# isl-org/adaptive-surface-reconstruction

Hardware: AMD Instinct MI355X
Metric: input points/sec to signed implicit values (higher is better)
Workload: dtype f32 via bf16x3 (24-bit operands, f32 accumulate)

## Files before the change

### adaptive-surface-reconstruction_amd/csrc/asr_common.h

```cpp
#pragma once
#include <hip/hip_runtime.h>

#include <cstdint>
#include <cstdio>
#include <map>
#include <string>
#include <tuple>
#include <vector>

#include "../../include/asr_hip.h"

typedef uint64_t u64;
typedef int64_t i64;
typedef uint32_t u32;

struct Arena {
    struct Slab {
        char* base;
        size_t size, used;
    };
    std::vector<Slab> slabs;
    size_t min_slab = size_t(256) << 20;
    size_t cap = 0;

// ... 44 lines not shown
    float* centers = nullptr;
    float* sizes = nullptr;
    int32_t* nidx = nullptr;
    uint8_t* nkidx = nullptr;
    i64* nrs = nullptr;
    int32_t* up_idx = nullptr;
    uint8_t* up_kidx = nullptr;
    i64* up_rs = nullptr;
    int32_t* down_idx = nullptr;
    uint8_t* down_kidx = nullptr;
    i64* down_rs = nullptr;
    int32_t* perm_nb = nullptr;
    int32_t* perm_up = nullptr;
    int32_t* perm_down = nullptr;
};

struct AsrOptions {
    i64 sconv_min_blocks = 2816;
    i64 sconv16_min_blocks = 1024;
    i64 sconv_wide_min = 2048;
    i64 row_segment = 524288;
    i64 search_hash_level = -1;
    i64 knn_deep = 1;
    i64 knn_cells = 1;
    i64 plan_arena = 0;
    i64 sconv_plan = 1;
    i64 row_ranked = 1;
    i64 row_lpt = 1;
    i64 overlap = 1;
    i64 cconv_valu = 0;
    i64 build_search = 1;
    i64 shard_geometry = -1;
    i64 shard_timing = 0;
    i64 search_priority = 2;
    i64 search_half = 1;
    i64 early_cells = 1;
    i64 early_sort = 1;
    i64 arena_cap_mb = 0;
    i64 inject_failure = 0;
    i64 sconv_split_min_rows = 2048;
    i64 sconv_split_rows = 32768;
};

struct asr_conv_plan_view {
    const uint4* hdr;
    const int32_t* pool;
    i64 groups;
    unsigned pool_bytes;
};
struct asr_conv_plan {
    uint4* hdr = nullptr;
    int32_t* pool = nullptr;
    i64 groups = 0, groups_pad = 0, blocks = 0;
    i64* offs = nullptr;
    const int32_t* nidx = nullptr;
    const uint8_t* kidx = nullptr;
    const i64* rs = nullptr;
    const int32_t* perm = nullptr;
    i64 num_out = 0;
    int K = 0;
    bool usable() const { return hdr && blocks * 64 < (i64(1) << 32) - 65536; }
    asr_conv_plan_view view() const { return {hdr, pool, groups, (unsigned)(blocks * 64)}; }
};

struct AsrPointIndex {
    bool valid = false;
    const float* pts = nullptr;
    const float* radii = nullptr;
    i64 n = 0;
    int lsort = 0;
    float4* sorted = nullptr;
    int32_t* ids = nullptr;
    int32_t* rank = nullptr;
    float* srad = nullptr;
    u64* codes = nullptr;
    u64* tab_keys = nullptr;
    u64 tab_mask = 0;
    int32_t* tab_start = nullptr;
    int32_t* tab_end = nullptr;
    int tab_lmin = 0, tab_lmax = -1, tab_lhash = 0, tab_grow = 0;
};

struct asr_hip_context {
    hipStream_t stream = nullptr;
    std::string err;
    AsrOptions opt;
    std::map<const void*, asr_conv_plan> conv_plans;
    std::map<std::string, i64> sconv_launches;
    ArenaMark build_mark;
    bool build_mark_ok = false;
    Arena persist;
    Arena scratch;
    Arena plan_arena;
    uint64_t plan_arena_epoch = 0;
    u64* nodes = nullptr;
    u64* leaves = nullptr;
    i64 num_nodes = 0, num_leaves = 0;
    asr_octree_frame frame;
    asr_implicit_sizes sizes;
    GridDev grids[ASR_NUM_GRIDS];
    int32_t* agg_idx = nullptr;
    float* agg_dist = nullptr;
    float* agg_compat = nullptr;
    i64* agg_rs = nullptr;
    int32_t* agg_spos = nullptr;
    const float4* agg_sorted = nullptr;
    bool has_search = false;
    bool build_sharded = false;
    const int32_t* agg_rows = nullptr;
    i64 agg_nq = 0;
    const float* agg_qcenters = nullptr;
    const float* agg_qsizes = nullptr;
// ... 293 lines not shown
```

### adaptive-surface-reconstruction_amd/csrc/asr_geom.hip

```cpp
#include <cstdlib>
#include <cstring>
#include <algorithm>
#include <rocprim/rocprim.hpp>

#include "asr_common.h"
#include "asr_prim.h"

namespace {
using namespace asr_prim;

constexpr int BLK = 256;

struct HashTab {
    u64* keys;
    int32_t* vals;
    u64 mask;
};

struct TabProbe {
    u64 bucket, step, low, bmask;
    __device__ inline u64 slot() const { return ((bucket & bmask) << 6) | low; }
    __device__ inline void next() { bucket += step; }
};
__device__ inline TabProbe tab_probe(const HashTab& t, u64 key) {
// ... 598 lines not shown
__global__ void k_gather_radii(const float* radii, const int32_t* ids, i64 n, float* out) {
    i64 i = blockIdx.x * (i64)blockDim.x + threadIdx.x;
    if (i < n) out[i] = radii[ids[i]];
}
__device__ inline int query_level(const asr_octree_frame& f, float r) {
    int lev = 0;
    while (lev < ASR_MAX_LEVEL && f.voxel_size[lev + 1] >= r) ++lev;
    return lev;
}
__global__ __launch_bounds__(256) void k_query_levels(asr_octree_frame f, const float* sizes, i64 v, int* cnt) {
    __shared__ int s_lo[4], s_hi[4];
    int lo = ASR_MAX_LEVEL, hi = 0;
    for (i64 i = blockIdx.x * (i64)blockDim.x + threadIdx.x; i < v; i += (i64)gridDim.x * blockDim.x) {
        const int l = query_level(f, sizes[i]);
        lo = min(lo, l);
        hi = max(hi, l);
    }
#pragma unroll
    for (int o = 32; o > 0; o >>= 1) {
        lo = min(lo, __shfl_xor(lo, o, 64));
        hi = max(hi, __shfl_xor(hi, o, 64));
    }
    if ((threadIdx.x & 63) == 0) {
        s_lo[threadIdx.x >> 6] = lo;
        s_hi[threadIdx.x >> 6] = hi;
    }
    __syncthreads();
    if (threadIdx.x == 0) {
        atomicMin(&cnt[6], min(min(s_lo[0], s_lo[1]), min(s_lo[2], s_lo[3])));
        atomicMax(&cnt[7], max(max(s_hi[0], s_hi[1]), max(s_hi[2], s_hi[3])));
    }
}
template <bool COUNT_ONLY>
__global__ __launch_bounds__(256) void k_cell_bounds(const u64* codes, i64 n, int lmin, int lmax, HashTab t,
                                                     int32_t* start, int32_t* end, int* cnt, int* level_cnt) {
    __shared__ int s_sum[4];
    __shared__ int s_lvl[ASR_MAX_LEVEL + 1];
    if (COUNT_ONLY) {
        if (threadIdx.x <= ASR_MAX_LEVEL) s_lvl[threadIdx.x] = 0;
        __syncthreads();
    }
    int local = 0;
    for (i64 i = blockIdx.x * (i64)blockDim.x + threadIdx.x; i <= n; i += (i64)gridDim.x * blockDim.x) {
        u64 a = i > 0 ? codes[i - 1] : 0, b = i < n ? codes[i] : 0;
        for (int l = lmin; l <= lmax; ++l) {
            int s = 3 * (ASR_MAX_LEVEL - l);
            u64 pa = (s >= 63) ? 0 : (a >> s), pb = (s >= 63) ? 0 : (b >> s);
            bool has_a = i > 0, has_b = i < n;
            if (has_a && has_b && pa == pb) continue;
            u64 marker = u64(1) << (3 * l);
            if (COUNT_ONLY) {
                if (has_b) {
                    ++local;
                    atomicAdd(&s_lvl[l], 1);
                }
            } else {
                u64 slot;
                if (has_a) {
                    if (tab_insert(t, pa | marker, &slot) < 0)
                        cnt[1] = 1;
                    else
                        end[slot] = (int32_t)i;
                }
                if (has_b) {
                    if (tab_insert(t, pb | marker, &slot) < 0)
                        cnt[1] = 1;
                    else
                        start[slot] = (int32_t)i;
                }
            }
        }
    }
    if (COUNT_ONLY) {
#pragma unroll
        for (int o = 32; o > 0; o >>= 1) local += __shfl_xor(local, o, 64);
        if ((threadIdx.x & 63) == 0) s_sum[threadIdx.x >> 6] = local;
        __syncthreads();
        if (threadIdx.x == 0) atomicAdd(&cnt[8], s_sum[0] + s_sum[1] + s_sum[2] + s_sum[3]);
        if (level_cnt && threadIdx.x <= ASR_MAX_LEVEL && s_lvl[threadIdx.x]) atomicAdd(&level_cnt[threadIdx.x], s_lvl[threadIdx.x]);
    }
}

__device__ inline float sqdist3(float ax, float ay, float az, float bx, float by, float bz) {
    float dx = ax - bx, dy = ay - by, dz = az - bz;
    float s = dx * dx;
    s = s + dy * dy;
    s = s + dz * dz;
    return s;
}

constexpr int RADIUS_LIGHT = 128;
constexpr int RADIUS_GIANT = 4096;
constexpr int RADIUS_SPLIT = 64;

struct CellIndex {
    HashTab tab;
    const int32_t* start;
    const int32_t* end;
    const u64* codes;
    int n;
    int lhash;
};
__device__ inline void cell_range(const CellIndex& ci, u64 cell, int lev, int& b, int& cnt) {
    b = 0;
    cnt = 0;
    if (lev <= ci.lhash) {
        const i64 slot = tab_find_slot(ci.tab, cell | (u64(1) << (3 * lev)));
        if (slot >= 0) {
            b = ci.start[slot];
            cnt = ci.end[slot] - b;
        }
        return;
    }
    const int s = 3 * (ASR_MAX_LEVEL - lev);
    int lo = 0, hi = ci.n;
    while (lo < hi) {
        const int mid = (lo + hi) >> 1;
        if ((ci.codes[mid] >> s) < cell)
            lo = mid + 1;
        else
            hi = mid;
    }
    int lo2 = lo, hi2 = ci.n;
    while (lo2 < hi2) {
        const int mid = (lo2 + hi2) >> 1;
        if ((ci.codes[mid] >> s) <= cell)
            lo2 = mid + 1;
        else
            hi2 = mid;
    }
    b = lo;
    cnt = lo2 - lo;
}

template <int NCELL>
__device__ inline int cells_prefix(int b, int n, int lane, int* s_pref, int* s_beg) {
    int pre = n;
#pragma unroll
    for (int o = 1; o < (NCELL > 32 ? 64 : 32); o <<= 1) {
        int up = __shfl_up(pre, o, 64);
        if (lane >= o) pre += up;
    }
    if (lane < NCELL) {
        s_pref[lane + 1] = pre;
        s_beg[lane] = b;
    }
    if (lane == 0) s_pref[0] = 0;
    const int total = __shfl(pre, NCELL - 1, 64);
    __builtin_amdgcn_wave_barrier();
    return total;
}
__device__ inline int radius_cells(const asr_octree_frame& f, const CellIndex& ci, float cx, float cy, float cz,
                                   float r, int lane, int* s_pref, int* s_beg) {
    const int lev = query_level(f, r);
    int x, y, z;
    frame_coord(f, cx, cy, cz, lev, x, y, z);
    const int lim = (1 << lev) - 1;
    int b = 0, n = 0;
    if (lane < 27) {
        int xx = x + lane % 3 - 1, yy = y + (lane / 3) % 3 - 1, zz = z + lane / 9 - 1;
        if (xx >= 0 && yy >= 0 && zz >= 0 && xx <= lim && yy <= lim && zz <= lim)
            cell_range(ci, asr_morton3d((u64)xx, (u64)yy, (u64)zz), lev, b, n);
    }
    return cells_prefix<27>(b, n, lane, s_pref, s_beg);
}

constexpr int EXTRA_CAP = 1 << 16;
struct AlignedQ {
    const u64* keys;
    const int2* extras;
    const int* extras_cnt;
    int lhalf_max;
};
__device__ inline int aligned_cells(const CellIndex& ci, const AlignedQ& aq, u64 key, int lane, int* s_pref, int* s_beg) {
    int x, y, z, lev;
    asr_key_coord(key, x, y, z, lev);
    int b = 0, n = 0;
    if (lev <= aq.lhalf_max) {
        const int lim = (2 << lev) - 1;
        const int xx = 2 * x - 1 + (lane & 3), yy = 2 * y - 1 + ((lane >> 2) & 3), zz = 2 * z - 1 + (lane >> 4);
        if (xx >= 0 && yy >= 0 && zz >= 0 && xx <= lim && yy <= lim && zz <= lim)
            cell_range(ci, asr_morton3d((u64)xx, (u64)yy, (u64)zz), lev + 1, b, n);
    } else if (lane < 27) {
        const int lim = (1 << lev) - 1;
        const int xx = x + lane % 3 - 1, yy = y + (lane / 3) % 3 - 1, zz = z + lane / 9 - 1;
        if (xx >= 0 && yy >= 0 && zz >= 0 && xx <= lim && yy <= lim && zz <= lim)
            cell_range(ci, asr_morton3d((u64)xx, (u64)yy, (u64)zz), lev, b, n);
    }
    return cells_prefix<64>(b, n, lane, s_pref, s_beg);
}
template <int NCELL = 27>
__device__ inline float4 radius_candidate(const float4* sorted, const int* s_pref, const int* s_beg, int i,
                                          int* pos_out = nullptr) {
    int lo = 0, hi = NCELL;
    while (hi - lo > 1) {
        int mid = (lo + hi) >> 1;
        if (s_pref[mid] <= i)
            lo = mid;
        else
            hi = mid;
    }
    const int pos = s_beg[lo] + (i - s_pref[lo]);
    if (pos_out) *pos_out = pos;
    return sorted[pos];
}

struct ExtraParams {
    int lmin, lmax;
    int T;
    int rho[ASR_MAX_LEVEL + 1];
};
__global__ void k_radius_extras(const u64* codes, const float4* sorted, i64 n, const u64* keys, i64 v, const float* centers,
                                const float* sizes, ExtraParams ep, int2* out, int* out_cnt) {
    const i64 s = blockIdx.x * (i64)blockDim.x + threadIdx.x;
    if (s >= n) return;
// ... 642 lines not shown
                            const int i = i0 + lane;
                            bool b2 = false;
                            if (i < total) {
                                const float4 pt = cand_pt(i);
                                b2 = __float_as_uint(sqdist3(pt.x, pt.y, pt.z, me.x, me.y, me.z)) == kth_bits &&
                                     (u32)__float_as_int(pt.w) < trial;
                            }
                            below += __popcll(__ballot(b2));
                        }
                        if (below < admit) idx_hi = trial;
                    }
                    votes_eq = 0;
                    for (int i0 = 0; i0 < total; i0 += 64) {
                        const int i = i0 + lane;
                        bool v = false;
                        if (i < total) {
                            const float4 pt = cand_pt(i);
                            v = __float_as_uint(sqdist3(pt.x, pt.y, pt.z, me.x, me.y, me.z)) == kth_bits &&
                                (u32)__float_as_int(pt.w) <= idx_hi && radii_in[__float_as_int(pt.w)] < thr;
                        }
                        votes_eq += __popcll(__ballot(v));
                    }
                }
                const int votes = votes_lt + votes_eq;
                if (lane == 0) inlier_out[__float_as_int(me.w)] = votes < outlier_threshold ? 1 : 0;
            }
            break;
        }
    }
    if (lane == 0 && radii_out) radii_out[__float_as_int(me.w)] = sqrtf(__uint_as_float(kth_bits));
}


__global__ void k_max_cell_pop(HashTab t, const int32_t* start, const int32_t* end, int level, int* out) {
    const u64 slot = blockIdx.x * (u64)blockDim.x + threadIdx.x;
    if (slot > t.mask) return;
    const u64 key = t.keys[slot];
    if (key == 0 || asr_key_level(key) != level) return;
    const int pop = end[slot] - start[slot];
    if (pop > KNN_CROWD) atomicMax(out, pop);
}

__global__ __launch_bounds__(256) void k_cell_list(const u64* codes, i64 n, int level, int32_t* list, int* cnt) {
    __shared__ int s_cnt[256];
    __shared__ int s_base;
    const int s = 3 * (ASR_MAX_LEVEL - level);
    const i64 base = blockIdx.x * (i64)4096;
    int mine = 0;
    unsigned flags = 0;
#pragma unroll
    for (int j = 0; j < 16; ++j) {
        const i64 i = base + j * 256 + threadIdx.x;
        if (i < n && (i == 0 || (codes[i - 1] >> s) != (codes[i] >> s))) {
            flags |= 1u << j;
            ++mine;
        }
    }
    s_cnt[threadIdx.x] = mine;
    __syncthreads();
    if (threadIdx.x == 0) {
        int tot = 0;
        for (int t = 0; t < 256; ++t) {
            const int c = s_cnt[t];
            s_cnt[t] = tot;
            tot += c;
        }
        s_base = tot ? atomicAdd(cnt, tot) : 0;
    }
    __syncthreads();
    int o = s_base + s_cnt[threadIdx.x];
#pragma unroll
    for (int j = 0; j < 16; ++j)
        if (flags & (1u << j)) list[o++] = (int32_t)(base + j * 256 + threadIdx.x);
}

constexpr int KNN_CELL_MAX_WORK = 12288;
template <int K>
__global__ __launch_bounds__(256) void k_knn_cells(asr_octree_frame f, const float4* sorted, i64 n, HashTab t,
                                                   const int32_t* start, const int32_t* end, int lfine, int k,
                                                   const int32_t* cells, i64 ncells, float* radii_out,
                                                   int32_t* fallback, int* fallback_cnt) {
    __shared__ int s_pref[4][28];
    __shared__ int s_beg[4][28];
    __shared__ __attribute__((aligned(16))) float4 s_cand[4][64];
    const int lane = threadIdx.x & 63, wave = threadIdx.x >> 6;
    const i64 ci = blockIdx.x * (i64)4 + wave;
    if (ci >= ncells) return;
    const int first = cells[ci];
    const float4 p0 = sorted[first];
    int x, y, z;
    frame_coord(f, p0.x, p0.y, p0.z, lfine, x, y, z);
    const int lim = (1 << lfine) - 1;
    x = min(max(x, 0), lim);
    y = min(max(y, 0), lim);
    z = min(max(z, 0), lim);
    int b = 0, cnt = 0;
    if (lane < 27) {
        constexpr unsigned char order[27] = {13, 4, 10, 12, 14, 16, 22, 1, 3, 5, 7, 9, 11, 15, 17, 19, 21, 23, 25,
                                             0, 2, 6, 8, 18, 20, 24, 26};
        const int c = order[lane];
        int xx = x + c % 3 - 1, yy = y + (c / 3) % 3 - 1, zz = z + c / 9 - 1;
        if (xx >= 0 && yy >= 0 && zz >= 0 && xx <= lim && yy <= lim && zz <= lim) {
            i64 slot = tab_find_slot(t, asr_morton3d((u64)xx, (u64)yy, (u64)zz) | (u64(1) << (3 * lfine)));
            if (slot >= 0) {
                b = start[slot];
                cnt = end[slot] - b;
            }
        }
    }
    int pre = cnt;
#pragma unroll
    for (int o = 1; o < 32; o <<= 1) {
        int up = __shfl_up(pre, o, 64);
        if (lane >= o) pre += up;
    }
    const int total = __shfl(pre, 26, 64);
    const int qb = __shfl(b, 0, 64), qn = __shfl(cnt, 0, 64);
    if (lane < 27) {
        s_pref[wave][lane + 1] = pre;
        s_beg[wave][lane] = b;
    }
    if (lane == 0) s_pref[wave][0] = 0;
    __builtin_amdgcn_wave_barrier();
    const float cs = f.voxel_size[lfine];
    const float cs2 = cs * cs;
    if (total < k || (i64)((qn + 63) / 64) * total > KNN_CELL_MAX_WORK) {
        for (int q0 = lane; q0 < qn; q0 += 64) fallback[atomicAdd(fallback_cnt, 1)] = qb + q0;
        return;
    }
    for (int q0 = 0; q0 < qn; q0 += 64) {
        const bool active = q0 + lane < qn;
        const float4 me = sorted[qb + (active ? q0 + lane : 0)];
        float a[K];
#pragma unroll
        for (int c = 0; c < K; ++c) a[c] = __uint_as_float(0x7f800000u);
        if (total >= k) {
            for (int c0 = 0; c0 < total; c0 += 64) {
                const int m = min(64, total - c0);
                __builtin_amdgcn_wave_barrier();
// ... 863 lines not shown
    *out_keys = arena_alloc<u64>(keep, vo);
    *up_idx = arena_alloc<int32_t>(keep, v);
    *up_kidx = arena_alloc<uint8_t>(keep, v);
    *up_rs = arena_alloc<i64>(keep, v + 1);
    *down_idx = arena_alloc<int32_t>(keep, v);
    *down_kidx = arena_alloc<uint8_t>(keep, v);
    *down_rs = arena_alloc<i64>(keep, vo + 1);
    if (!src || !*out_keys || !*up_idx || !*up_kidx || !*up_rs || !*down_idx || !*down_kidx || !*down_rs)
        ASR_FAIL(ctx, ASR_HIP_EHIP, "arena allocation failed");
    return coarsen_lists(ctx, keys, v, pre, vo, src, *out_keys, *up_idx, *up_kidx, *up_rs, *down_idx, *down_kidx,
                         *down_rs);
}

int asr_geom_voxel_info(asr_hip_context* ctx, const asr_octree_frame* frame, const u64* keys,
                        i64 v, float* centers, float* sizes) {
    if (v <= 0) return ASR_HIP_OK;
    k_voxel_info<<<grid_for(v, BLK), BLK, 0, ctx->stream>>>(*frame, keys, v, centers, sizes);
    ASR_CHECK_LAUNCH(ctx);
    return ASR_HIP_OK;
}

struct RadiusState {
    bool valid = false;
    asr_octree_frame frame;
    float4* sorted = nullptr;
    int32_t* ids = nullptr;
    int32_t* rank = nullptr;
    const u64* codes = nullptr;
    u64* codes_w = nullptr;
    const u64* codes_u = nullptr;
    const int32_t* ids_u = nullptr;
    int32_t* ids_w = nullptr;
    int lhash = ASR_MAX_LEVEL;
    CellIndex index() const { return {tab, start, end, codes, (int)n, lhash}; }
    HashTab tab;
    int32_t* start = nullptr;
    int32_t* end = nullptr;
    i64 n = 0, v = 0;
    u64* tmp = nullptr;
    int32_t* heavy = nullptr;
    uint8_t* is_heavy = nullptr;
    i64 num_heavy = 0;
    int* hc_pref = nullptr;
    int* hc_beg = nullptr;
    const u64* dual_leaves = nullptr;
    i64 dual_nl = 0;
    float* srad = nullptr;
    const float* radii_src = nullptr;
    int lsort = 0;
    int cell_grow = 0;
    bool aligned = false;
    bool aligned_main = false;
    AlignedQ aq = {nullptr, nullptr, nullptr, -1};
};
static RadiusState& rstate(asr_hip_context* ctx) {
    if (!ctx->radius_state) ctx->radius_state = new RadiusState();
    return *(RadiusState*)ctx->radius_state;
}
void asr_geom_release(asr_hip_context* ctx) {
    delete (RadiusState*)ctx->radius_state;
    ctx->radius_state = nullptr;
}

static int sort_points(asr_hip_context* ctx, const asr_octree_frame* frame, const float* pts, i64 n, int lsort,
                       RadiusState& st, Arena* keep, bool want_rank, const float* radii, bool keep_all = false) {
    st.frame = *frame;
    st.n = n;
    st.lsort = lsort;
    Arena& ka = keep ? *keep : ctx->scratch;
    u64* codes_u = arena_alloc<u64>(ctx->scratch, n + 1);
    u64* codes = arena_alloc<u64>(keep_all ? ka : ctx->scratch, n + 1);
    int32_t* ids_u = arena_alloc<int32_t>(ctx->scratch, n + 1);
    int32_t* ids = arena_alloc<int32_t>(ka, n + 1);
    st.sorted = arena_alloc<float4>(ka, n + 1);
    st.ids = ids;
    st.codes = codes;
    st.codes_w = codes;
    st.codes_u = codes_u;
    st.ids_u = ids_u;
    st.ids_w = ids;
    st.rank = want_rank ? arena_alloc<int32_t>(ka, n + 1) : nullptr;
    st.srad = radii ? arena_alloc<float>(keep_all ? ka : ctx->scratch, n + 1) : nullptr;
    st.radii_src = radii;
    if (!codes_u || !codes || !ids_u || !ids || !st.sorted || (want_rank && !st.rank) || (radii && !st.srad))
        ASR_FAIL(ctx, ASR_HIP_EHIP, "arena allocation failed");
    if (n > 0) {
        k_point_codes<<<grid_for(n, BLK), BLK, 0, ctx->stream>>>(*frame, pts, n, codes_u, ids_u, ctx->d_flags);
        ASR_CHECK_LAUNCH(ctx);
        ASR_TRY((sort_pairs<u64, int32_t>(ctx, ctx->scratch, codes_u, codes, ids_u, ids, n, 63,
                                          3 * (ASR_MAX_LEVEL - std::max(lsort, 1)))));
        k_gather_points<<<grid_for(n, BLK), BLK, 0, ctx->stream>>>(pts, ids, n, st.sorted, st.rank, radii, st.srad);
        ASR_CHECK_LAUNCH(ctx);
    }
    return ASR_HIP_OK;
}
static int build_cell_table(asr_hip_context* ctx, i64 n, int lmin, int lmax, RadiusState& st, bool hash_all,
                            Arena* where = nullptr);
static int build_point_index(asr_hip_context* ctx, const asr_octree_frame* frame, const float* pts,
                             i64 n, int lmin, int lmax, RadiusState& st, Arena* keep = nullptr,
                             bool want_rank = false, bool hash_all = true, const float* radii = nullptr) {
    ASR_TRY(fresh_flags(ctx));
    ASR_TRY(sort_points(ctx, frame, pts, n, lmax, st, keep, want_rank, radii));
    return build_cell_table(ctx, n, lmin, lmax, st, hash_all);
}
static int build_cell_table(asr_hip_context* ctx, i64 n, int lmin, int lmax, RadiusState& st, bool hash_all, Arena* where) {
    Arena& arena = where ? *where : ctx->scratch;
    int host[16];
    const u64* codes = st.codes;
    HashTab dummy{nullptr, nullptr, 0};
    int* level_cnt = ctx->d_flags + 32;
    int host_lvl[ASR_MAX_LEVEL + 1] = {0};
    if (n > 0) {
        ASR_HIP_CHECK(ctx, hipMemsetAsync(level_cnt, 0, (ASR_MAX_LEVEL + 1) * sizeof(int), ctx->stream));
        k_cell_bounds<true><<<std::min<unsigned>(grid_for(n + 1, BLK), 4096u), BLK, 0, ctx->stream>>>(
                codes, n, lmin, lmax, dummy, nullptr, nullptr, ctx->d_flags, level_cnt);
        ASR_CHECK_LAUNCH(ctx);
        ASR_HIP_CHECK(ctx, hipMemcpyAsync(host_lvl, level_cnt, sizeof(host_lvl), hipMemcpyDeviceToHost, ctx->stream));
    }
    ASR_TRY(read_flags(ctx, host));
    if (host[11]) ASR_FAIL(ctx, ASR_HIP_EINVAL, "points contain non-finite values");
    int lhash = lmax;
    if (!hash_all) {
        lhash = lmin;
        while (lhash < lmax && (i64)host_lvl[lhash + 1] * 2 <= n) ++lhash;
        if (ctx->opt.search_hash_level >= 0) lhash = (int)std::min<i64>(lmax, std::max<i64>(lmin - 1, ctx->opt.search_hash_level));
    }
    st.lhash = lhash;
    i64 cells = 0;
    for (int l = lmin; l <= lhash; ++l) cells += host_lvl[l];
    u64 cap = next_pow2((u64)std::max<i64>(1024, 2 * cells)) << st.cell_grow;
    ASR_TRY(make_table(ctx, arena, cap, false, st.tab));
    st.start = arena_alloc<int32_t>(arena, cap);
    st.end = arena_alloc<int32_t>(arena, cap);
    if (!st.start || !st.end) ASR_FAIL(ctx, ASR_HIP_EHIP, "arena allocation failed");
    if (n > 0) {
        k_cell_bounds<false><<<grid_for(n + 1, BLK), BLK, 0, ctx->stream>>>(
                codes, n, lmin, lhash, st.tab, st.start, st.end, ctx->d_flags, nullptr);
        ASR_CHECK_LAUNCH(ctx);
    }
    return ASR_HIP_OK;
}

constexpr int PRESORT_LEVEL = 13;
__global__ __launch_bounds__(256) void k_finest_point_level(asr_octree_frame f, const float* __restrict__ radii, i64 n,
                                                            float radius_scale, int max_depth, int* __restrict__ out) {
    int m = 0;
    for (i64 i = blockIdx.x * (i64)blockDim.x + threadIdx.x; i < n; i += (i64)gridDim.x * blockDim.x) {
        int l = level_from_scale(f, radius_scale * radii[i]);
        l = l < max_depth ? l : max_depth;
        m = max(m, l);
    }
#pragma unroll
    for (int o = 32; o > 0; o >>= 1) m = max(m, __shfl_xor(m, o, 64));
    if ((threadIdx.x & 63) == 0 && m > 0) atomicMax(out, m);
}
int asr_geom_presort(asr_hip_context* ctx, Arena& keep, const asr_octree_frame* frame, const float* pts,
                     const float* radii, i64 n, float radius_scale, int max_depth) {
    ASR_TRY(ensure_flags(ctx));
    AsrPointIndex& pi = ctx->pindex;
    pi.valid = false;
    if (n <= 0 || n >= (i64(1) << 31)) return ASR_HIP_OK;
    int lsort = PRESORT_LEVEL;
    if (radius_scale > 0.f && radii) {
        int host[16];
        ASR_TRY(fresh_flags(ctx));
        k_finest_point_level<<<std::min<unsigned>(grid_for(n, BLK), 2048u), BLK, 0, ctx->stream>>>(
                *frame, radii, n, radius_scale, std::min(max_depth, ASR_MAX_LEVEL), ctx->d_flags + 8);
        ASR_CHECK_LAUNCH(ctx);
        ASR_TRY(read_flags(ctx, host));
        lsort = std::max(PRESORT_LEVEL, std::min(ASR_MAX_LEVEL, host[8] + 1));
    }
    RadiusState st;
    ASR_TRY(sort_points(ctx, frame, pts, n, lsort, st, &keep, true, radii, true));
    pi.pts = pts;
    pi.radii = radii;
    pi.n = n;
    pi.lsort = lsort;
    pi.sorted = st.sorted;
    pi.ids = st.ids;
    pi.rank = st.rank;
    pi.srad = st.srad;
    pi.codes = st.codes_w;
    pi.valid = true;
    return ASR_HIP_OK;
}

int asr_geom_precells(asr_hip_context* ctx, Arena& keep) {
    AsrPointIndex& pi = ctx->pindex;
    pi.tab_keys = nullptr;
    if (!pi.valid || pi.n <= 0) return ASR_HIP_OK;
    RadiusState st;
    st.codes = st.codes_w = pi.codes;
    st.n = pi.n;
    st.cell_grow = rstate(ctx).cell_grow;
    ASR_TRY(fresh_flags(ctx));
    ASR_TRY(build_cell_table(ctx, pi.n, 1, pi.lsort, st, false, &keep));
    int host[16];
    ASR_TRY(read_flags(ctx, host));
    if (host[1]) return ASR_HIP_OK;
    pi.tab_grow = st.cell_grow;
    pi.tab_keys = st.tab.keys;
    pi.tab_mask = st.tab.mask;
    pi.tab_start = st.start;
    pi.tab_end = st.end;
    pi.tab_lmin = 1;
    pi.tab_lmax = pi.lsort;
    pi.tab_lhash = st.lhash;
    return ASR_HIP_OK;
}

static int query_level_range(asr_hip_context* ctx, const asr_octree_frame* frame, const float* sizes,
                             i64 v, int* lmin, int* lmax) {
    int host[16];
    ASR_TRY(fresh_flags(ctx));
    int init[2] = {ASR_MAX_LEVEL, 0};
    ASR_HIP_CHECK(ctx, hipMemcpyAsync(ctx->d_flags + 6, init, 2 * sizeof(int),
                                      hipMemcpyHostToDevice, ctx->stream));
    k_query_levels<<<std::min<unsigned>(grid_for(v, BLK), 2048u), BLK, 0, ctx->stream>>>(*frame, sizes, v, ctx->d_flags);
    ASR_CHECK_LAUNCH(ctx);
    ASR_TRY(read_flags(ctx, host));
    *lmin = host[6];
    *lmax = host[7];
    return ASR_HIP_OK;
}

int asr_geom_radius_count(asr_hip_context* ctx, const asr_octree_frame* frame, const float* pts,
                          i64 n, const float* centers, const float* sizes, i64 v, i64* rs,
                          i64* num_pairs, Arena* keep, const float* radii, const u64* voxel_keys, int lmin_hint,
                          int lmax_hint, const AsrPointIndex* pre) {
    ASR_TRY(ensure_flags(ctx));
    RadiusState& st = rstate(ctx);
    st.valid = false;
    if (v <= 0) {
        *num_pairs = 0;
        if (rs) ASR_HIP_CHECK(ctx, hipMemsetAsync(rs, 0, sizeof(i64), ctx->stream));
        return ASR_HIP_OK;
    }
    if (n >= (i64(1) << 31)) ASR_FAIL(ctx, ASR_HIP_EINVAL, "too many points for int32 indices");
    int host[16];
    st.v = v;
    int lmin = lmin_hint, lmax = lmax_hint;
    if (lmin < 0 || lmax < lmin) ASR_TRY(query_level_range(ctx, frame, sizes, v, &lmin, &lmax));
    st.aligned = voxel_keys != nullptr && ctx->opt.search_half != 0;
    st.aligned_main = st.aligned && ctx->opt.search_half >= 2;
    ExtraParams ep;
    memset(&ep, 0, sizeof(ep));
    int lhalf_max = -1;
    if (st.aligned) {
        double M = 1;
        for (int d = 0; d < 3; ++d)
            M = std::max(M, std::max(std::fabs((double)frame->offset[d]), std::fabs((double)(1 << ASR_MAX_LEVEL) - frame->offset[d])));
        const int T = 2 + (int)std::floor(3.0 * (M + 1) / 16777216.0);
        lhalf_max = ASR_MAX_LEVEL - 1;
        while (lhalf_max >= 0 && (1 << (ASR_MAX_LEVEL - 1 - lhalf_max)) < 16 * T) --lhalf_max;
        ep.T = T;
        ep.lmin = lmin;
        ep.lmax = std::min(lmax, lhalf_max);
        for (int l = 0; l <= ASR_MAX_LEVEL; ++l)
            ep.rho[l] = (int)std::ceil(std::sqrt(2.0 * (double)(1 << (ASR_MAX_LEVEL - l)) * T)) + 2 * T + 1;
    }
    const int ltab = st.aligned ? std::min(ASR_MAX_LEVEL, std::min(lmax, lhalf_max) + 1) : lmax;
    if (pre && pre->valid && pre->pts == pts && pre->n == n && pre->lsort >= std::max(lmax, ltab) && (!radii || pre->srad)) {
        st.frame = *frame;
        st.n = n;
        st.lsort = pre->lsort;
        st.sorted = pre->sorted;
        st.ids = pre->ids;
        st.rank = pre->rank;
        st.srad = radii ? pre->srad : nullptr;
        st.radii_src = radii;
        st.codes = st.codes_w = pre->codes;
        st.codes_u = nullptr;
        st.ids_u = nullptr;
        st.ids_w = pre->ids;
        ASR_TRY(fresh_flags(ctx));
        if (pre->tab_keys && pre->tab_grow == st.cell_grow && pre->tab_lmin <= lmin && pre->tab_lmax >= std::max(lmax, ltab)) {
            st.tab = HashTab{pre->tab_keys, nullptr, pre->tab_mask};
            st.start = pre->tab_start;
            st.end = pre->tab_end;
            st.lhash = pre->tab_lhash;
        } else {
            ASR_TRY(build_cell_table(ctx, n, lmin, std::max(lmax, ltab), st, false));
        }
    } else {
        ASR_TRY(build_point_index(ctx, frame, pts, n, lmin, std::max(lmax, ltab), st, keep, true, false, radii));
    }
    i64* counts = arena_alloc<i64>(ctx->scratch, v + 1);
    st.tmp = arena_alloc<u64>(ctx->scratch, (size_t)v * RADIUS_LIGHT);
    st.heavy = arena_alloc<int32_t>(ctx->scratch, v);
    st.is_heavy = arena_alloc<uint8_t>(ctx->scratch, v);
    int2* extras = arena_alloc<int2>(ctx->scratch, EXTRA_CAP);
    if (!counts || !st.tmp || !st.heavy || !st.is_heavy || !extras) ASR_FAIL(ctx, ASR_HIP_EHIP, "arena allocation failed");
    ASR_HIP_CHECK(ctx, hipMemsetAsync(ctx->d_flags + 10, 0, sizeof(int), ctx->stream));
    ASR_HIP_CHECK(ctx, hipMemsetAsync(ctx->d_flags + 15, 0, sizeof(int), ctx->stream));
    st.aq = AlignedQ{voxel_keys, extras, ctx->d_flags + 15, lhalf_max};
    if (st.aligned && ep.lmax >= ep.lmin && n > 0) {
        k_radius_extras<<<grid_for(n, BLK), BLK, 0, ctx->stream>>>(st.codes, st.sorted, n, voxel_keys, v, centers, sizes,
                                                                  ep, extras, ctx->d_flags + 15);
        ASR_CHECK_LAUNCH(ctx);
    }
    const unsigned qgrid = grid_for(v + 1, 4);
    if (st.aligned_main)
        k_radius_query<2, true><<<qgrid, BLK, 0, ctx->stream>>>(*frame, st.sorted, centers, sizes, v, st.index(), st.aq, counts,
                                                                st.tmp, st.heavy, ctx->d_flags + 10, st.is_heavy);
    else
        k_radius_query<2, false><<<qgrid, BLK, 0, ctx->stream>>>(*frame, st.sorted, centers, sizes, v, st.index(), st.aq, counts,
                                                                 st.tmp, st.heavy, ctx->d_flags + 10, st.is_heavy);
    ASR_CHECK_LAUNCH(ctx);
    ASR_TRY(read_flags(ctx, host));
    if (host[1]) {
        if (st.cell_grow >= 6) ASR_FAIL(ctx, ASR_HIP_ELOGIC, "radius search cell table overflow");
        st.cell_grow += 2;
        return asr_geom_radius_count(ctx, frame, pts, n, centers, sizes, v, rs, num_pairs, keep, radii, voxel_keys,
                                     lmin_hint, lmax_hint, pre);
    }
    if (host[15] > EXTRA_CAP) ASR_FAIL(ctx, ASR_HIP_ELOGIC, "radius search: %d pairs in the rounding margin (cap %d)", host[15], EXTRA_CAP);
    ctx->search_extras = host[15];
    st.num_heavy = host[10];
    if (st.num_heavy > 0) {
        st.hc_pref = arena_alloc<int>(ctx->scratch, (size_t)st.num_heavy * HC_LD);
        st.hc_beg = arena_alloc<int>(ctx->scratch, (size_t)st.num_heavy * HC_LD);
        if (!st.hc_pref || !st.hc_beg) ASR_FAIL(ctx, ASR_HIP_EHIP, "arena allocation failed");
        const unsigned cgrid = grid_for(st.num_heavy, 4);
        if (st.aligned) {
            k_radius_heavy_cells<true><<<cgrid, BLK, 0, ctx->stream>>>(*frame, centers, sizes, st.heavy, (int)st.num_heavy,
                                                                       st.index(), st.aq, st.hc_pref, st.hc_beg);
            k_radius_heavy<false, true><<<dim3((unsigned)st.num_heavy, RADIUS_SPLIT), BLK, 0, ctx->stream>>>(
                    *frame, st.sorted, centers, sizes, st.heavy, st.index(), st.aq, counts, nullptr, nullptr, nullptr, nullptr,
                    st.hc_pref, st.hc_beg, 0);
        } else {
            k_radius_heavy_cells<false><<<cgrid, BLK, 0, ctx->stream>>>(*frame, centers, sizes, st.heavy, (int)st.num_heavy,
                                                                        st.index(), st.aq, st.hc_pref, st.hc_beg);
            k_radius_heavy<false, false><<<dim3((unsigned)st.num_heavy, RADIUS_SPLIT), BLK, 0, ctx->stream>>>(
                    *frame, st.sorted, centers, sizes, st.heavy, st.index(), st.aq, counts, nullptr, nullptr, nullptr, nullptr,
                    st.hc_pref, st.hc_beg, 0);
// ... 72 lines not shown
        case 4: ASR_ATTR_BLEND(4); break;
        case 8: ASR_ATTR_BLEND(8); break;
        default: ASR_ATTR_BLEND(16); break;
    }
#undef ASR_ATTR_BLEND
    ASR_CHECK_LAUNCH(ctx);
    return ASR_HIP_OK;
}

static int deepen_point_index(asr_hip_context* ctx, const float* pts, RadiusState& st, int ldeep) {
    ASR_TRY((sort_pairs<u64, int32_t>(ctx, ctx->scratch, st.codes_u, st.codes_w, st.ids_u, st.ids_w, st.n, 63,
                                      3 * (ASR_MAX_LEVEL - ldeep))));
    k_gather_points<<<grid_for(st.n, BLK), BLK, 0, ctx->stream>>>(pts, st.ids_w, st.n, st.sorted, st.rank);
    ASR_CHECK_LAUNCH(ctx);
    return ASR_HIP_OK;
}

int asr_geom_knn(asr_hip_context* ctx, const asr_octree_frame* frame, const float* pts, i64 n, int k,
                 const float* radii_in, float radius_fraction, int outlier_threshold, float* radii_out,
                 uint8_t* inlier_out) {
    ASR_TRY(ensure_flags(ctx));
    if (n <= 0) return ASR_HIP_OK;
    if (k < 1) ASR_FAIL(ctx, ASR_HIP_EINVAL, "knn: k must be >= 1");
    if (n >= (i64(1) << 31)) ASR_FAIL(ctx, ASR_HIP_EINVAL, "too many points for int32 indices");
    int lfine = 1;
    while (lfine < ASR_MAX_LEVEL - 1 && (i64(1) << (3 * lfine)) < n) ++lfine;
    RadiusState st;
    int host[16];
    ASR_TRY(build_point_index(ctx, frame, pts, n, 0, lfine, st));
    st.lhash = lfine;
    int ldeep = lfine;
    {
        ASR_HIP_CHECK(ctx, hipMemsetAsync(ctx->d_flags + 14, 0, sizeof(int), ctx->stream));
        k_max_cell_pop<<<grid_for((i64)st.tab.mask + 1, BLK), BLK, 0, ctx->stream>>>(st.tab, st.start, st.end, lfine,
                                                                                   ctx->d_flags + 14);
        ASR_CHECK_LAUNCH(ctx);
        ASR_TRY(read_flags(ctx, host));
        if (host[14] > KNN_CROWD && ctx->opt.knn_deep) {
            ldeep = std::min<int>(ASR_MAX_LEVEL, lfine + 8);
            ASR_TRY(deepen_point_index(ctx, pts, st, ldeep));
        }
    }
    const bool fast = !inlier_out && radii_out && k <= 32 && n >= k && ctx->opt.knn_cells;
    if (fast) {
        int32_t* cells = arena_alloc<int32_t>(ctx->scratch, n + 1);
        int32_t* fallback = arena_alloc<int32_t>(ctx->scratch, n + 1);
        if (!cells || !fallback) ASR_FAIL(ctx, ASR_HIP_EHIP, "arena allocation failed");
        ASR_HIP_CHECK(ctx, hipMemsetAsync(ctx->d_flags + 12, 0, 2 * sizeof(int), ctx->stream));
        k_cell_list<<<grid_for(n, 4096), BLK, 0, ctx->stream>>>(st.codes, n, lfine, cells, ctx->d_flags + 12);
        ASR_CHECK_LAUNCH(ctx);
        ASR_TRY(read_flags(ctx, host));
        const i64 ncells = host[12];
#define ASR_KNN_CELLS(K_)                                                                                           \
    k_knn_cells<K_><<<grid_for(ncells, 4), BLK, 0, ctx->stream>>>(*frame, st.sorted, n, st.tab, st.start, st.end, lfine, \
                                                                   k, cells, ncells, radii_out, fallback,            \
                                                                   ctx->d_flags + 13)
        if (k <= 8)
            ASR_KNN_CELLS(8);
        else if (k <= 16)
            ASR_KNN_CELLS(16);
        else if (k <= 24)
            ASR_KNN_CELLS(24);
        else
            ASR_KNN_CELLS(32);
#undef ASR_KNN_CELLS
        ASR_CHECK_LAUNCH(ctx);
        ASR_TRY(read_flags(ctx, host));
        const i64 nfb = host[13];
        if (nfb > 0) {
            k_knn<<<grid_for(nfb, 4), BLK, 0, ctx->stream>>>(*frame, st.sorted, n, st.index(), lfine, ldeep, k, radii_in,
                                                             radius_fraction, outlier_threshold, radii_out, nullptr,
                                                             fallback, nfb);
            ASR_CHECK_LAUNCH(ctx);
        }
    } else {
        k_knn<<<grid_for(n, 4), BLK, 0, ctx->stream>>>(*frame, st.sorted, n, st.index(), lfine, ldeep, k, radii_in,
                                                       radius_fraction, outlier_threshold, radii_out, inlier_out,
                                                       nullptr, 0);
        ASR_CHECK_LAUNCH(ctx);
    }
    ASR_TRY(read_flags(ctx, host));
    if (host[1]) ASR_FAIL(ctx, ASR_HIP_ELOGIC, "cell table overflow");
    return ASR_HIP_OK;
}

int asr_geom_radius_fill(asr_hip_context* ctx, const float* pts, const float* radii, i64 n,
                         const float* centers, const float* sizes, i64 v, const i64* rs,
// ... 66 lines not shown
}

int asr_geom_dual_count(asr_hip_context* ctx, const u64* nodes, i64 nn, const u64* leaves, i64 nl, i64* num_cells) {
    ASR_TRY(ensure_flags(ctx));
    *num_cells = 0;
    RadiusState& st0 = rstate(ctx);
    st0.dual_leaves = leaves;
    st0.dual_nl = nl;
    if (nl <= 0) return ASR_HIP_OK;
    ctx->scratch.reset();
    HashTab t;
    u64 cap = next_pow2((u64)std::max<i64>(1024, 2 * nn));
    ASR_TRY(make_table(ctx, ctx->scratch, cap, true, t));
    ASR_HIP_CHECK(ctx, hipMemsetAsync(t.vals, 0xFF, cap * sizeof(int32_t), ctx->stream));
    ASR_TRY(fresh_flags(ctx));
    int32_t* keep = t.vals;
    t.vals = arena_alloc<int32_t>(ctx->scratch, cap);
    if (!t.vals) ASR_FAIL(ctx, ASR_HIP_EHIP, "arena allocation failed");
    k_map_build<<<grid_for(nn, BLK), BLK, 0, ctx->stream>>>(nodes, nn, t, ctx->d_flags);
    ASR_CHECK_LAUNCH(ctx);
    t.vals = keep;
    k_map_build<<<grid_for(nl, BLK), BLK, 0, ctx->stream>>>(leaves, nl, t, ctx->d_flags);
    ASR_CHECK_LAUNCH(ctx);
    i64* counts = arena_alloc<i64>(ctx->scratch, nl + 1);
    i64* offsets = arena_alloc<i64>(ctx->scratch, nl + 1);
    if (!counts || !offsets) ASR_FAIL(ctx, ASR_HIP_EHIP, "arena allocation failed");
    k_dual_count<<<grid_for(nl + 1, BLK), BLK, 0, ctx->stream>>>(leaves, nl, t, counts);
    ASR_CHECK_LAUNCH(ctx);
    ASR_TRY(scan_counts(ctx, ctx->scratch, counts, offsets, nl + 1));
    ASR_TRY(read_i64(ctx, offsets + nl, num_cells));
    RadiusState& st = rstate(ctx);
    st.valid = false;
    st.tab = t;
    st.start = (int32_t*)offsets;
    st.v = -nl;
    return ASR_HIP_OK;
}
int asr_geom_dual_fill(asr_hip_context* ctx, i64* out) {
    RadiusState& st = rstate(ctx);
    const i64 nl = st.dual_nl;
    if (nl <= 0) return ASR_HIP_OK;
    if (st.v != -nl) ASR_FAIL(ctx, ASR_HIP_EINVAL, "dual_fill must follow the matching dual_count call");
    int host[16];
    k_dual_fill<<<grid_for(nl, BLK), BLK, 0, ctx->stream>>>(st.dual_leaves, nl, st.tab, (const i64*)st.start, out,
                                                            ctx->d_flags);
    ASR_CHECK_LAUNCH(ctx);
    ASR_TRY(read_flags(ctx, host));
    st.v = 0;
    if (host[1]) ASR_FAIL(ctx, ASR_HIP_ELOGIC, "invalid key after searching for node (cpp/lib/grid.cpp:435-440)");
    return ASR_HIP_OK;
}

int asr_geom_invert(asr_hip_context* ctx, i64 num_points, const int32_t* idx, const i64* rs,
                    i64 num_rows, const uint8_t* attr, int32_t* out_idx, i64* out_rs,
                    uint8_t* out_attr, i64 known_pairs) {
    i64 p = known_pairs;
    if (p < 0) {
        p = 0;
        if (num_rows > 0) ASR_TRY(read_i64(ctx, rs + num_rows, &p));
    }
    i64* counts = arena_alloc<i64>(ctx->scratch, num_points + 1);
    if (!counts) ASR_FAIL(ctx, ASR_HIP_EHIP, "arena allocation failed");
    ASR_HIP_CHECK(ctx, hipMemsetAsync(counts, 0, (num_points + 1) * sizeof(i64), ctx->stream));
    if (p > 0) {
        k_invert_hist<<<grid_for(p, BLK), BLK, 0, ctx->stream>>>(idx, p, counts, num_points);
        ASR_CHECK_LAUNCH(ctx);
    }
    ASR_TRY(scan_counts(ctx, ctx->scratch, counts, out_rs, num_points + 1));
    if (p > 0) {
        int32_t* src = arena_alloc<int32_t>(ctx->scratch, p);
        int32_t* src_s = arena_alloc<int32_t>(ctx->scratch, p);
        int32_t* key_s = arena_alloc<int32_t>(ctx->scratch, p);
        if (!src || !src_s || !key_s) ASR_FAIL(ctx, ASR_HIP_EHIP, "arena allocation failed");
        k_iota32<<<grid_for(p, BLK), BLK, 0, ctx->stream>>>(src, p);
        ASR_CHECK_LAUNCH(ctx);
        ASR_TRY((sort_pairs<int32_t, int32_t>(ctx, ctx->scratch, idx, key_s, src, src_s, p,
                                              bits_for(num_points + 1))));
// ... 235 lines not shown
```

Baseline: 272.7 million.

## Pack cell start/end with per-child counts and derive child ranges from parents

Replaces separate start/end arrays of the cell hash table with a 16-byte record holding start, end and eight per-child population counts, filled during cell-bound construction and by a new child-count kernel. The aligned radius query can then resolve half-cell child ranges by looking up the 27 parent cells and prefix-summing child counts via lane shuffles, instead of 64 separate hash probes. The aligned query path is now used whenever search_half is set, and search_priority defaults change. It adds table-build work and memory, and falls back to direct probes when counts saturate.

```diff
diff --git a/adaptive-surface-reconstruction_amd/csrc/asr_common.h b/adaptive-surface-reconstruction_amd/csrc/asr_common.h
--- a/adaptive-surface-reconstruction_amd/csrc/asr_common.h
+++ b/adaptive-surface-reconstruction_amd/csrc/asr_common.h
@@ -100,7 +100,7 @@
     i64 build_search = 1;
     i64 shard_geometry = -1;
     i64 shard_timing = 0;
-    i64 search_priority = 2;
+    i64 search_priority = 1;
     i64 search_half = 1;
     i64 early_cells = 1;
     i64 early_sort = 1;
@@ -131,6 +131,12 @@
     asr_conv_plan_view view() const { return {hdr, pool, groups, (unsigned)(blocks * 64)}; }
 };
 
+struct AsrCellRec {
+    int32_t start, end;
+    uint8_t cnt[8];
+};
+static_assert(sizeof(AsrCellRec) == 16, "one 16-byte load per cell");
+
 struct AsrPointIndex {
     bool valid = false;
     const float* pts = nullptr;
@@ -144,8 +150,7 @@
     u64* codes = nullptr;
     u64* tab_keys = nullptr;
     u64 tab_mask = 0;
-    int32_t* tab_start = nullptr;
-    int32_t* tab_end = nullptr;
+    AsrCellRec* tab_rec = nullptr;
     int tab_lmin = 0, tab_lmax = -1, tab_lhash = 0, tab_grow = 0;
 };
 
diff --git a/adaptive-surface-reconstruction_amd/csrc/asr_geom.hip b/adaptive-surface-reconstruction_amd/csrc/asr_geom.hip
--- a/adaptive-surface-reconstruction_amd/csrc/asr_geom.hip
+++ b/adaptive-surface-reconstruction_amd/csrc/asr_geom.hip
@@ -654,8 +654,8 @@
     }
 }
 template <bool COUNT_ONLY>
-__global__ __launch_bounds__(256) void k_cell_bounds(const u64* codes, i64 n, int lmin, int lmax, HashTab t,
-                                                     int32_t* start, int32_t* end, int* cnt, int* level_cnt) {
+__global__ __launch_bounds__(256) void k_cell_bounds(const u64* codes, i64 n, int lmin, int lmax, int lsort, HashTab t,
+                                                     AsrCellRec* rec, int* cnt, int* level_cnt) {
     __shared__ int s_sum[4];
     __shared__ int s_lvl[ASR_MAX_LEVEL + 1];
     if (COUNT_ONLY) {
@@ -665,10 +665,12 @@
     int local = 0;
     for (i64 i = blockIdx.x * (i64)blockDim.x + threadIdx.x; i <= n; i += (i64)gridDim.x * blockDim.x) {
         u64 a = i > 0 ? codes[i - 1] : 0, b = i < n ? codes[i] : 0;
+        const bool has_a = i > 0, has_b = i < n;
+        u64 slot_b = 0;
+        bool top = false;
         for (int l = lmin; l <= lmax; ++l) {
             int s = 3 * (ASR_MAX_LEVEL - l);
             u64 pa = (s >= 63) ? 0 : (a >> s), pb = (s >= 63) ? 0 : (b >> s);
-            bool has_a = i > 0, has_b = i < n;
             if (has_a && has_b && pa == pb) continue;
             u64 marker = u64(1) << (3 * l);
             if (COUNT_ONLY) {
@@ -682,15 +684,35 @@
                     if (tab_insert(t, pa | marker, &slot) < 0)
                         cnt[1] = 1;
                     else
-                        end[slot] = (int32_t)i;
+                        rec[slot].end = (int32_t)i;
                 }
                 if (has_b) {
-                    if (tab_insert(t, pb | marker, &slot) < 0)
+                    if (tab_insert(t, pb | marker, &slot) < 0) {
                         cnt[1] = 1;
-                    else
-                        start[slot] = (int32_t)i;
+                    } else {
+                        rec[slot].start = (int32_t)i;
+                        if (l == lmax) {
+                            slot_b = slot;
+                            top = true;
+                            if (lmax >= lsort) *reinterpret_cast<u64*>(rec[slot].cnt) = ~u64(0);
+                        }
+                    }
                 }
             }
+        }
+        if (!COUNT_ONLY && top && lmax < lsort) {
+            const int sc = 3 * (ASR_MAX_LEVEL - (lmax + 1));
+            const u64 cell = b >> (sc + 3);
+            u64 counts = 0, c = b >> sc;
+            int run = 0;
+            bool more;
+            do {
+                counts += u64(1) << (8 * (c & 7));
+                ++run;
+                more = i + run < n && ((c = codes[i + run] >> sc) >> 3) == cell;
+            } while (more && run < 254);
+            if (more) counts |= ~u64(0) << (8 * (c & 7));
+            *reinterpret_cast<u64*>(rec[slot_b].cnt) = counts;
         }
     }
     if (COUNT_ONLY) {
@@ -701,6 +723,17 @@
         if (threadIdx.x == 0) atomicAdd(&cnt[8], s_sum[0] + s_sum[1] + s_sum[2] + s_sum[3]);
         if (level_cnt && threadIdx.x <= ASR_MAX_LEVEL && s_lvl[threadIdx.x]) atomicAdd(&level_cnt[threadIdx.x], s_lvl[threadIdx.x]);
     }
+}
+__global__ __launch_bounds__(256) void k_cell_children(HashTab t, AsrCellRec* rec, int lmin) {
+    const u64 slot = blockIdx.x * (u64)blockDim.x + threadIdx.x;
+    if (slot > t.mask) return;
+    const u64 key = t.keys[slot];
+    if (key == 0) return;
+    const int l = asr_key_level(key);
+    if (l <= lmin) return;
+    const int2 se = *reinterpret_cast<const int2*>(&rec[slot]);
+    const i64 parent = tab_find_slot(t, ((key ^ (u64(1) << (3 * l))) >> 3) | (u64(1) << (3 * (l - 1))));
+    if (parent >= 0) rec[parent].cnt[key & 7] = (uint8_t)min(se.y - se.x, 255);
 }
 
 __device__ inline float sqdist3(float ax, float ay, float az, float bx, float by, float bz) {
@@ -717,8 +750,7 @@
 
 struct CellIndex {
     HashTab tab;
-    const int32_t* start;
-    const int32_t* end;
+    const AsrCellRec* rec;
     const u64* codes;
     int n;
     int lhash;
@@ -729,8 +761,9 @@
     if (lev <= ci.lhash) {
         const i64 slot = tab_find_slot(ci.tab, cell | (u64(1) << (3 * lev)));
         if (slot >= 0) {
-            b = ci.start[slot];
-            cnt = ci.end[slot] - b;
+            const int2 se = *reinterpret_cast<const int2*>(&ci.rec[slot]);
+            b = se.x;
+            cnt = se.y - b;
         }
         return;
     }
@@ -793,6 +826,7 @@
     const int2* extras;
     const int* extras_cnt;
     int lhalf_max;
+    int from_parents;
 };
 __device__ inline int aligned_cells(const CellIndex& ci, const AlignedQ& aq, u64 key, int lane, int* s_pref, int* s_beg) {
     int x, y, z, lev;
@@ -800,9 +834,41 @@
     int b = 0, n = 0;
     if (lev <= aq.lhalf_max) {
         const int lim = (2 << lev) - 1;
-        const int xx = 2 * x - 1 + (lane & 3), yy = 2 * y - 1 + ((lane >> 2) & 3), zz = 2 * z - 1 + (lane >> 4);
-        if (xx >= 0 && yy >= 0 && zz >= 0 && xx <= lim && yy <= lim && zz <= lim)
-            cell_range(ci, asr_morton3d((u64)xx, (u64)yy, (u64)zz), lev + 1, b, n);
+        const int hx = lane & 3, hy = (lane >> 2) & 3, hz = lane >> 4;
+        const int xx = 2 * x - 1 + hx, yy = 2 * y - 1 + hy, zz = 2 * z - 1 + hz;
+        const bool inside = xx >= 0 && yy >= 0 && zz >= 0 && xx <= lim && yy <= lim && zz <= lim;
+        bool direct = inside;
+        if (aq.from_parents && lev <= ci.lhash) {
+            int4 r = make_int4(0, 0, 0, 0);
+            if (lane < 27) {
+                const int px = x + lane % 3 - 1, py = y + (lane / 3) % 3 - 1, pz = z + lane / 9 - 1;
+                const int plim = (1 << lev) - 1;
+                if (px >= 0 && py >= 0 && pz >= 0 && px <= plim && py <= plim && pz <= plim) {
+                    const i64 slot = tab_find_slot(ci.tab, asr_morton3d((u64)px, (u64)py, (u64)pz) | (u64(1) << (3 * lev)));
+                    if (slot >= 0) r = *reinterpret_cast<const int4*>(&ci.rec[slot]);
+                }
+            }
+            const int parent = ((hx + 1) >> 1) + 3 * ((hy + 1) >> 1) + 9 * ((hz + 1) >> 1);
+            const int start = __shfl(r.x, parent, 64);
+            const u64 cnts = (u64)(u32)__shfl(r.z, parent, 64) | ((u64)(u32)__shfl(r.w, parent, 64) << 32);
+            const int c = ((hx + 1) & 1) | (((hy + 1) & 1) << 1) | (((hz + 1) & 1) << 2);
+            int before = 0;
+            bool known = true;
+#pragma unroll
+            for (int j = 0; j < 8; ++j) {
+                const int cj = (int)((cnts >> (8 * j)) & 255);
+                if (j <= c) known = known && cj != 255;
+                if (j < c) before += cj;
+                if (j == c) n = cj;
+            }
+            if (known) {
+                b = start + before;
+                direct = false;
+            } else {
+                n = 0;
+            }
+        }
+        if (direct) cell_range(ci, asr_morton3d((u64)xx, (u64)yy, (u64)zz), lev + 1, b, n);
     } else if (lane < 27) {
         const int lim = (1 << lev) - 1;
         const int xx = x + lane % 3 - 1, yy = y + (lane / 3) % 3 - 1, zz = z + lane / 9 - 1;
@@ -1511,12 +1577,12 @@
 }
 
 
-__global__ void k_max_cell_pop(HashTab t, const int32_t* start, const int32_t* end, int level, int* out) {
+__global__ void k_max_cell_pop(HashTab t, const AsrCellRec* rec, int level, int* out) {
     const u64 slot = blockIdx.x * (u64)blockDim.x + threadIdx.x;
     if (slot > t.mask) return;
     const u64 key = t.keys[slot];
     if (key == 0 || asr_key_level(key) != level) return;
-    const int pop = end[slot] - start[slot];
+    const int pop = rec[slot].end - rec[slot].start;
     if (pop > KNN_CROWD) atomicMax(out, pop);
 }
 
@@ -1556,7 +1622,7 @@
 constexpr int KNN_CELL_MAX_WORK = 12288;
 template <int K>
 __global__ __launch_bounds__(256) void k_knn_cells(asr_octree_frame f, const float4* sorted, i64 n, HashTab t,
-                                                   const int32_t* start, const int32_t* end, int lfine, int k,
+                                                   const AsrCellRec* rec, int lfine, int k,
                                                    const int32_t* cells, i64 ncells, float* radii_out,
                                                    int32_t* fallback, int* fallback_cnt) {
     __shared__ int s_pref[4][28];
@@ -1582,8 +1648,9 @@
         if (xx >= 0 && yy >= 0 && zz >= 0 && xx <= lim && yy <= lim && zz <= lim) {
             i64 slot = tab_find_slot(t, asr_morton3d((u64)xx, (u64)yy, (u64)zz) | (u64(1) << (3 * lfine)));
             if (slot >= 0) {
-                b = start[slot];
-                cnt = end[slot] - b;
+                const int2 se = *reinterpret_cast<const int2*>(&rec[slot]);
+                b = se.x;
+                cnt = se.y - b;
             }
         }
     }
@@ -2513,10 +2580,10 @@
     const int32_t* ids_u = nullptr;
     int32_t* ids_w = nullptr;
     int lhash = ASR_MAX_LEVEL;
-    CellIndex index() const { return {tab, start, end, codes, (int)n, lhash}; }
+    CellIndex index() const { return {tab, rec, codes, (int)n, lhash}; }
     HashTab tab;
-    int32_t* start = nullptr;
-    int32_t* end = nullptr;
+    AsrCellRec* rec = nullptr;
+    const i64* dual_offsets = nullptr;
     i64 n = 0, v = 0;
     u64* tmp = nullptr;
     int32_t* heavy = nullptr;
@@ -2531,8 +2598,7 @@
     int lsort = 0;
     int cell_grow = 0;
     bool aligned = false;
-    bool aligned_main = false;
-    AlignedQ aq = {nullptr, nullptr, nullptr, -1};
+    AlignedQ aq = {nullptr, nullptr, nullptr, -1, 0};
 };
 static RadiusState& rstate(asr_hip_context* ctx) {
     if (!ctx->radius_state) ctx->radius_state = new RadiusState();
@@ -2594,7 +2660,7 @@
     if (n > 0) {
         ASR_HIP_CHECK(ctx, hipMemsetAsync(level_cnt, 0, (ASR_MAX_LEVEL + 1) * sizeof(int), ctx->stream));
         k_cell_bounds<true><<<std::min<unsigned>(grid_for(n + 1, BLK), 4096u), BLK, 0, ctx->stream>>>(
-                codes, n, lmin, lmax, dummy, nullptr, nullptr, ctx->d_flags, level_cnt);
+                codes, n, lmin, lmax, st.lsort, dummy, nullptr, ctx->d_flags, level_cnt);
         ASR_CHECK_LAUNCH(ctx);
         ASR_HIP_CHECK(ctx, hipMemcpyAsync(host_lvl, level_cnt, sizeof(host_lvl), hipMemcpyDeviceToHost, ctx->stream));
     }
@@ -2610,14 +2676,19 @@
     i64 cells = 0;
     for (int l = lmin; l <= lhash; ++l) cells += host_lvl[l];
     u64 cap = next_pow2((u64)std::max<i64>(1024, 2 * cells)) << st.cell_grow;
-    ASR_TRY(make_table(ctx, arena, cap, false, st.tab));
-    st.start = arena_alloc<int32_t>(arena, cap);
-    st.end = arena_alloc<int32_t>(arena, cap);
-    if (!st.start || !st.end) ASR_FAIL(ctx, ASR_HIP_EHIP, "arena allocation failed");
+    u64* block = arena_alloc<u64>(arena, 3 * cap);
+    if (!block) ASR_FAIL(ctx, ASR_HIP_EHIP, "arena allocation failed");
+    ASR_HIP_CHECK(ctx, hipMemsetAsync(block, 0, 3 * cap * sizeof(u64), ctx->stream));
+    st.tab = HashTab{block, nullptr, cap - 1};
+    st.rec = reinterpret_cast<AsrCellRec*>(block + cap);
     if (n > 0) {
         k_cell_bounds<false><<<grid_for(n + 1, BLK), BLK, 0, ctx->stream>>>(
-                codes, n, lmin, lhash, st.tab, st.start, st.end, ctx->d_flags, nullptr);
+                codes, n, lmin, lhash, st.lsort, st.tab, st.rec, ctx->d_flags, nullptr);
         ASR_CHECK_LAUNCH(ctx);
+        if (lhash > lmin) {
+            k_cell_children<<<grid_for((i64)cap, BLK), BLK, 0, ctx->stream>>>(st.tab, st.rec, lmin);
+            ASR_CHECK_LAUNCH(ctx);
+        }
     }
     return ASR_HIP_OK;
 }
@@ -2673,6 +2744,7 @@
     RadiusState st;
     st.codes = st.codes_w = pi.codes;
     st.n = pi.n;
+    st.lsort = pi.lsort;
     st.cell_grow = rstate(ctx).cell_grow;
     ASR_TRY(fresh_flags(ctx));
     ASR_TRY(build_cell_table(ctx, pi.n, 1, pi.lsort, st, false, &keep));
@@ -2682,8 +2754,7 @@
     pi.tab_grow = st.cell_grow;
     pi.tab_keys = st.tab.keys;
     pi.tab_mask = st.tab.mask;
-    pi.tab_start = st.start;
-    pi.tab_end = st.end;
+    pi.tab_rec = st.rec;
     pi.tab_lmin = 1;
     pi.tab_lmax = pi.lsort;
     pi.tab_lhash = st.lhash;
@@ -2723,7 +2794,6 @@
     int lmin = lmin_hint, lmax = lmax_hint;
     if (lmin < 0 || lmax < lmin) ASR_TRY(query_level_range(ctx, frame, sizes, v, &lmin, &lmax));
     st.aligned = voxel_keys != nullptr && ctx->opt.search_half != 0;
-    st.aligned_main = st.aligned && ctx->opt.search_half >= 2;
     ExtraParams ep;
     memset(&ep, 0, sizeof(ep));
     int lhalf_max = -1;
@@ -2757,8 +2827,7 @@
         ASR_TRY(fresh_flags(ctx));
         if (pre->tab_keys && pre->tab_grow == st.cell_grow && pre->tab_lmin <= lmin && pre->tab_lmax >= std::max(lmax, ltab)) {
             st.tab = HashTab{pre->tab_keys, nullptr, pre->tab_mask};
-            st.start = pre->tab_start;
-            st.end = pre->tab_end;
+            st.rec = pre->tab_rec;
             st.lhash = pre->tab_lhash;
         } else {
             ASR_TRY(build_cell_table(ctx, n, lmin, std::max(lmax, ltab), st, false));
@@ -2774,14 +2843,14 @@
     if (!counts || !st.tmp || !st.heavy || !st.is_heavy || !extras) ASR_FAIL(ctx, ASR_HIP_EHIP, "arena allocation failed");
     ASR_HIP_CHECK(ctx, hipMemsetAsync(ctx->d_flags + 10, 0, sizeof(int), ctx->stream));
     ASR_HIP_CHECK(ctx, hipMemsetAsync(ctx->d_flags + 15, 0, sizeof(int), ctx->stream));
-    st.aq = AlignedQ{voxel_keys, extras, ctx->d_flags + 15, lhalf_max};
+    st.aq = AlignedQ{voxel_keys, extras, ctx->d_flags + 15, lhalf_max, ctx->opt.search_half == 1};
     if (st.aligned && ep.lmax >= ep.lmin && n > 0) {
         k_radius_extras<<<grid_for(n, BLK), BLK, 0, ctx->stream>>>(st.codes, st.sorted, n, voxel_keys, v, centers, sizes,
                                                                   ep, extras, ctx->d_flags + 15);
         ASR_CHECK_LAUNCH(ctx);
     }
     const unsigned qgrid = grid_for(v + 1, 4);
-    if (st.aligned_main)
+    if (st.aligned)
         k_radius_query<2, true><<<qgrid, BLK, 0, ctx->stream>>>(*frame, st.sorted, centers, sizes, v, st.index(), st.aq, counts,
                                                                 st.tmp, st.heavy, ctx->d_flags + 10, st.is_heavy);
     else
@@ -2920,7 +2989,7 @@
     int ldeep = lfine;
     {
         ASR_HIP_CHECK(ctx, hipMemsetAsync(ctx->d_flags + 14, 0, sizeof(int), ctx->stream));
-        k_max_cell_pop<<<grid_for((i64)st.tab.mask + 1, BLK), BLK, 0, ctx->stream>>>(st.tab, st.start, st.end, lfine,
+        k_max_cell_pop<<<grid_for((i64)st.tab.mask + 1, BLK), BLK, 0, ctx->stream>>>(st.tab, st.rec, lfine,
                                                                                    ctx->d_flags + 14);
         ASR_CHECK_LAUNCH(ctx);
         ASR_TRY(read_flags(ctx, host));
@@ -2940,7 +3009,7 @@
         ASR_TRY(read_flags(ctx, host));
         const i64 ncells = host[12];
 #define ASR_KNN_CELLS(K_)                                                                                           \
-    k_knn_cells<K_><<<grid_for(ncells, 4), BLK, 0, ctx->stream>>>(*frame, st.sorted, n, st.tab, st.start, st.end, lfine, \
+    k_knn_cells<K_><<<grid_for(ncells, 4), BLK, 0, ctx->stream>>>(*frame, st.sorted, n, st.tab, st.rec, lfine, \
                                                                    k, cells, ncells, radii_out, fallback,            \
                                                                    ctx->d_flags + 13)
         if (k <= 8)
@@ -3073,7 +3142,7 @@
     RadiusState& st = rstate(ctx);
     st.valid = false;
     st.tab = t;
-    st.start = (int32_t*)offsets;
+    st.dual_offsets = offsets;
     st.v = -nl;
     return ASR_HIP_OK;
 }
@@ -3083,7 +3152,7 @@
     if (nl <= 0) return ASR_HIP_OK;
     if (st.v != -nl) ASR_FAIL(ctx, ASR_HIP_EINVAL, "dual_fill must follow the matching dual_count call");
     int host[16];
-    k_dual_fill<<<grid_for(nl, BLK), BLK, 0, ctx->stream>>>(st.dual_leaves, nl, st.tab, (const i64*)st.start, out,
+    k_dual_fill<<<grid_for(nl, BLK), BLK, 0, ctx->stream>>>(st.dual_leaves, nl, st.tab, st.dual_offsets, out,
                                                             ctx->d_flags);
     ASR_CHECK_LAUNCH(ctx);
     ASR_TRY(read_flags(ctx, host));
```

Result: no change. 273.7 million, median of 6 (+0.4%).
